# akanazawa/human_dynamics

Measured on AMD Instinct MI355X. Metric: frames/sec/GPU (ResNet+temporal+SMPL, 224x224); SMPL verts max-abs-err, higher is better.
Workload: dtype f16x3

## Files before the change

human_dynamics_amd/_lib.py:

```python
from __future__ import annotations

import ctypes as C
import os

from . import devflags

HERE = os.path.dirname(os.path.abspath(__file__))
LIB_PATH = devflags.get("LIB_PATH") or os.path.join(HERE, "libhmmr_hip.so")

HMMR_F32, HMMR_BF16, HMMR_F16X3 = 0, 1, 2
FLAG_SATURATED = 1
FLAG_NAN = 2
ABI_VERSION = 19
RESNET_UNITS = 16
RESNET_PROF_SLOTS = 64
MAX_TEMPORAL_BLOCKS = 8
MAX_REGRESSORS = 8

_vp, _fp, _ip = C.c_void_p, C.c_void_p, C.c_void_p


class ConvDesc(C.Structure):
    _fields_ = [
        ("in_", _vp), ("w", _vp), ("scale", _fp), ("shift", _fp), ("res", _vp), ("out", _vp),
# ... 2 lines not shown
        ("n_img", C.c_int), ("hin", C.c_int), ("win", C.c_int), ("cin", C.c_int),
        ("in_img_stride", C.c_int64), ("in_row_stride", C.c_int), ("in_px_stride", C.c_int),
        ("kh", C.c_int), ("kw", C.c_int), ("sy", C.c_int), ("sx", C.c_int), ("py", C.c_int), ("px", C.c_int),
        ("ho", C.c_int), ("wo", C.c_int), ("cout", C.c_int), ("ldo", C.c_int),
        ("ldr", C.c_int), ("res_strided", C.c_int), ("res_img_stride", C.c_int64),
        ("res_row_stride", C.c_int), ("res_px_stride", C.c_int),
        ("relu", C.c_int), ("tile", C.c_int),
        ("split_k", C.c_int), ("ws", _vp), ("ws_bytes", C.c_size_t),
        ("pro_scale", _fp), ("pro_shift", _fp),
        ("out_b", _vp), ("ldo_b", C.c_int), ("n_split", C.c_int), ("relu_b", C.c_int),
        ("in2", _vp), ("cin2", C.c_int), ("k_order", C.c_int),
        ("batch", C.c_int), ("batch_in_bytes", C.c_int64), ("batch_w_bytes", C.c_int64), ("batch_out_bytes", C.c_int64),
        ("batch_res_bytes", C.c_int64), ("batch_scale_bytes", C.c_int64), ("batch_shift_bytes", C.c_int64),
    ]


class TailDesc(C.Structure):
    _fields_ = [
        ("dtype", C.c_int), ("h2", _vp), ("m", C.c_int), ("c_mid", C.c_int), ("depth", C.c_int),
        ("w3", _vp), ("scale3", _fp), ("shift3", _fp),
        ("res", _vp), ("ldr", C.c_int), ("res_strided", C.c_int), ("res_img_stride", C.c_int64),
        ("res_row_stride", C.c_int), ("res_px_stride", C.c_int), ("ho", C.c_int), ("wo", C.c_int),
        ("out", _vp), ("pre_scale", _fp), ("pre_shift", _fp),
        ("w1", _vp), ("scale1", _fp), ("shift1", _fp), ("relu1", C.c_int), ("n2", C.c_int),
        ("out_h1", _vp),
        ("h1", _vp), ("hin", C.c_int), ("win", C.c_int), ("w2", _vp), ("scale2", _fp), ("shift2", _fp),
        ("xp", _vp), ("wsc", _vp), ("shift_sc", _fp),
        ("conv2_stride", C.c_int), ("out_pre", _vp),
        ("pair_stream", _vp), ("c_xp", C.c_int), ("unit_stream", _vp),
    ]


class Debug(C.Structure):
    _fields_ = [("stem_route", C.c_int), ("stem_no_conv1", C.c_int), ("gemm_probe", C.c_int), ("smpl_blend_mfma", C.c_int), ("ief_no_group", C.c_int), ("reserved", C.c_int * 3),
                ("pair_min_pixels", C.c_int), ("pair_two_tile_min", C.c_int), ("pair_form", C.c_int)]


class LaunchCounts(C.Structure):
    _fields_ = [("unit_pair", C.c_ulonglong), ("b1_unit", C.c_ulonglong), ("tail_split", C.c_ulonglong), ("conv3x3_stream", C.c_ulonglong),
                ("conv1x1_stream", C.c_ulonglong)]


class Layer(C.Structure):
    _fields_ = [("w", _vp), ("scale", _fp), ("shift", _fp), ("tile", C.c_int), ("k_order", C.c_int)]


class ResnetUnit(C.Structure):
    _fields_ = [("conv1", Layer), ("conv2", Layer), ("conv3", Layer), ("shortcut", Layer), ("c3sc", Layer), ("sc_c1", Layer),
                ("w3_frag", _vp), ("w1n_frag", _vp), ("pair_stream", _vp), ("conv1_frag", _vp), ("unit_stream", _vp), ("pre_scale", _fp), ("pre_shift", _fp),
                ("c_in", C.c_int), ("base", C.c_int), ("depth", C.c_int), ("stride", C.c_int),
                ("fuse_preact", C.c_int), ("fuse_tail", C.c_int)]


class ResnetWeights(C.Structure):
    _fields_ = [("dtype", C.c_int), ("stem", Layer),
                ("unit", ResnetUnit * RESNET_UNITS), ("post_scale", _fp), ("post_shift", _fp)]


class TemporalBlock(C.Structure):
    _fields_ = [("gn1_gamma", _fp), ("gn1_beta", _fp), ("conv1", Layer),
                ("gn2_gamma", _fp), ("gn2_beta", _fp), ("conv2", Layer)]


class TemporalWeights(C.Structure):
    _fields_ = [("dtype", C.c_int), ("num_blocks", C.c_int), ("block", TemporalBlock * MAX_TEMPORAL_BLOCKS)]


# ... 142 lines not shown
```

human_dynamics_amd/csrc/conv3x3_stream.hip:

```cpp
#include <type_traits>

#include "common.h"
#include "hmmr_hip.h"

namespace {

typedef const __attribute__((address_space(1))) void* gptr_t;
typedef __attribute__((address_space(3))) void* lptr_t;

__device__ u32x4 g_s3_dump[64 + 32];

struct S3Args {
    const char* in;
    const char* wstream;
    const float* scale; const float* shift;
    void* out; int ldo;
    int M, H, W, C, nc;
    int relu, tiles_n, n_tiles;
    long long nt_stride;
    unsigned long long* ts;
};

#ifndef S3_PROBE_BITS
#define S3_PROBE_BITS 0
#endif
#define S3_PROBE(bit) (((S3_PROBE_BITS) & (bit)) != 0)
#ifdef HMMR_GEMM_PROBE
#define S3_STAMP(k) do { if (a.ts) { const unsigned long long t_ = __builtin_amdgcn_s_memtime(); if ((threadIdx.x & 63) == 0) a.ts[(blockIdx.x * 4 + (threadIdx.x >> 6)) * 8 + (k)] = t_; } } while (0)
#else
#define S3_STAMP(k) do { } while (0)
#endif

template <int N> __device__ __forceinline__ void s3_wait() {
    static_assert(N >= 0 && N < 64, "vmcnt is a 6-bit counter");
    __builtin_amdgcn_s_waitcnt((N & 15) | (7 << 4) | (0 << 8) | ((N >> 4) << 14));
}

template <int OFF> __device__ __forceinline__ shalf8 s3_rd(unsigned addr) {
    shalf8 v; asm volatile("ds_read_b128 %0, %1 offset:%2" : "=v"(v) : "v"(addr), "n"(OFF)); return v;
}

struct xfrag { shalf8 hi, lo; };

constexpr int S3_NS = 6;

template <int V> using s3_ic = std::integral_constant<int, V>;

template <int FM, int FN, int WGM, int WGN, int WMAX, bool SPLIT = true>
__global__ __launch_bounds__(256, 1) void conv3x3_stream_kernel(const S3Args a) {
    constexpr int NP = SPLIT ? 3 : 2;
    constexpr int ESZ = SPLIT ? 4 : 2;
    constexpr int NB = WGN * FN;
    static_assert(WGM * WGN == 4 && (NB == 4 || NB == 2) && FM * FN <= 16, "4 waves, 128 or 64 channels, at most 16 accumulators");
    constexpr int R = WGM * FM, BM = 32 * R;
    constexpr int NPP = (BM + 2 * WMAX + 2 + 63) / 64;
    constexpr int NS = S3_NS, SLAB = NB * 2048, RING = NS * SLAB;
    constexpr int RW = NB / 2;
    constexpr int ZROWS = 32 * (FM - 1) + 16;
    constexpr int PBUF = (NPP * 64 + ZROWS) * 64;
    constexpr int NR = 2 * (FM + FN), NG = NP * FM * FN;
    static_assert(2048 * (FM - 1) + 16 < 65536, "instruction offsets");
    static_assert(NR <= NG - 4, "one fragment read per gap");

    extern __shared__ __attribute__((aligned(256))) char smem[];
    S3_STAMP(0);
    const int tid = threadIdx.x, lane = tid & 63;
    const int wave = __builtin_amdgcn_readfirstlane(tid >> 6);
    const int lr = lane & 31, lh = lane >> 5;
    const int L = xcd_remap(blockIdx.x, a.n_tiles);
    const int mt = L / a.tiles_n, nt = L - mt * a.tiles_n;
    const int m0 = mt * BM;
    const int W = a.W, HW = a.H * a.W;
    const int base = m0 - W - 1;
    const int nc = a.nc, nk = 9 * nc;
    const int wm = wave / WGN, wn = wave - wm * WGN;
    const unsigned lds0 = (unsigned)(unsigned long long)(lptr_t)smem;

    const char* pptr[NPP];
#pragma unroll
    for (int q = 0; q < NPP; ++q) {
        const int r = 64 * q + 16 * wave + (lane >> 2);
        int px = base + r;
        px = px < 0 ? 0 : (px >= a.M ? a.M - 1 : px);
        pptr[q] = a.in + ((long long)px * a.C) * ESZ + (((lane & 3) ^ ((r >> 2) & 3)) << 4);
        if (S3_PROBE(128)) pptr[q] = a.in + ((long long)(px & ~15) * a.C) * ESZ + lane * 16;
    }
    auto patch_piece = [&](int q, int c, int buf) {
        char* dst = smem + RING + buf * PBUF + wave * 1024;
        __builtin_amdgcn_global_load_lds((gptr_t)(pptr[q] + c * 64), (lptr_t)(dst + q * 4096), 16, 0, 0);
    };
    const char* gw = a.wstream + (long long)nt * a.nt_stride + wave * (RW * 1024) + lane * 16;
    auto ring_dma = [&](int s, int slot) {
        const char* src = gw + (long long)s * SLAB;
        char* dst = smem + slot * SLAB + wave * (RW * 1024);
        __builtin_amdgcn_global_load_lds((gptr_t)src, (lptr_t)dst, 16, 0, 0);
        if constexpr (RW == 2) __builtin_amdgcn_global_load_lds((gptr_t)src, (lptr_t)dst, 16, 1024, 0);
    };
#pragma unroll
    for (int q = 0; q < NPP; ++q) patch_piece(q, 0, 0);
#pragma unroll
    for (int s_ = 0; s_ < NS; ++s_) ring_dma(s_, s_);

    for (int i = tid; i < 2 * ZROWS * 4; i += 256) {
        const int pl = i / (ZROWS * 4), o = i - pl * (ZROWS * 4);
        *(u32x4*)(smem + RING + pl * PBUF + NPP * 64 * 64 + o * 16) = u32x4{0u, 0u, 0u, 0u};
    }
    {
        float* cst = (float*)(smem + RING + 2 * PBUF);
        if (tid < 64 * NB) cst[tid] = tid < 32 * NB ? a.scale[nt * (32 * NB) + tid] : a.shift[nt * (32 * NB) + tid - 32 * NB];
    }
    unsigned mtop[FM], mbot[FM], mlef[FM], mrig[FM];
#pragma unroll
    for (int i = 0; i < FM; ++i) {
        const int m = m0 + (wm * FM + i) * 32 + lr;
        const int rem = m % HW, y = rem / W, x = rem - y * W;
        mtop[i] = (unsigned)__builtin_amdgcn_ballot_w64(y == 0);
        mbot[i] = (unsigned)__builtin_amdgcn_ballot_w64(y == a.H - 1);
        mlef[i] = (unsigned)__builtin_amdgcn_ballot_w64(x == 0);
        mrig[i] = (unsigned)__builtin_amdgcn_ballot_w64(x == W - 1);
    }

    f32x16 acc[FM][FN];
#pragma unroll
    for (int i = 0; i < FM; ++i)
#pragma unroll
        for (int j = 0; j < FN; ++j) {
#pragma unroll
            for (int r = 0; r < 16; ++r) acc[i][j][r] = 0.f;
            asm volatile("" : "+a"(acc[i][j]));
        }

    const unsigned vW = lds0 + wn * FN * 2048 + lane * 16;
    const int rb0 = wm * FM * 32 + lr;
    const unsigned lh2 = SPLIT ? 2 * lh : lh;
    constexpr unsigned XL = SPLIT ? 16u : 32u;
    xfrag fx[2][FM];
    wfrag fw[2][FN];
    unsigned A0 = 0, A0l = 0, Zb = 0, Zbl = 0, adcur = 0, adcurl = 0;

    auto read_one = [&](auto tap_c, int set, int r, int slot_) {
        constexpr int TAP_ = decltype(tap_c)::value, KY = TAP_ / 3, KX = TAP_ % 3;
        if (r < 2 * FN) {
            const int j = r >> 1, pl = r & 1;
#define S3_F(SL, J, PL) if (slot_ == SL && j == J && pl == PL) { shalf8 v = s3_rd<SL * SLAB + J * 2048 + PL * 1024>(vW); if (PL) fw[set][J].lo = v; else fw[set][J].hi = v; }
#define S3_FJ(SL, J) S3_F(SL, J, 0) S3_F(SL, J, 1)
#define S3_FS(SL) S3_FJ(SL, 0) if constexpr (FN > 1) { S3_FJ(SL, 1) } if constexpr (FN > 2) { S3_FJ(SL, 2) S3_FJ(SL, 3) }
            S3_FS(0) S3_FS(1) S3_FS(2) S3_FS(3) S3_FS(4) S3_FS(5)
#undef S3_FS
#undef S3_FJ
#undef S3_F
        } else {
            const int i = (r - 2 * FN) >> 1, pl = (r - 2 * FN) & 1;
            if (pl == 0) {
                if (KY == 1 && KX == 1) { adcur = A0; adcurl = A0l; }
                else {
                    const int ii = i < FM ? i : 0;
                    const unsigned my = KY == 0 ? mtop[ii] : (KY == 2 ? mbot[ii] : 0u);
                    const unsigned mx = KX == 0 ? mlef[ii] : (KX == 2 ? mrig[ii] : 0u);
                    asm volatile("s_mov_b32 vcc_lo, %2\n\ts_mov_b32 vcc_hi, %2\n\tv_cndmask_b32 %0, %3, %4, vcc\n\tv_cndmask_b32 %1, %5, %6, vcc"
                                 : "=&v"(adcur), "=v"(adcurl) : "s"(my | mx), "v"(A0), "v"(Zb), "v"(A0l), "v"(Zbl) : "vcc");
                }
            }
#define S3_X(I) if constexpr (I < FM) { if (i == I) { if (pl) fx[set][I].lo = s3_rd<I * 2048>(adcurl); else fx[set][I].hi = s3_rd<I * 2048>(adcur); } }
            S3_X(0) S3_X(1) S3_X(2) S3_X(3) S3_X(4) S3_X(5) S3_X(6) S3_X(7) S3_X(8) S3_X(9) S3_X(10) S3_X(11) S3_X(12) S3_X(13) S3_X(14) S3_X(15)
#undef S3_X
        }
    };
    auto tap_setup = [&](auto tap_c, int buf_) {
        constexpr int TAP_ = decltype(tap_c)::value, KY = TAP_ / 3, KX = TAP_ % 3;
        const unsigned rowp = (unsigned)(rb0 + KY * W + KX);
        const unsigned ph = (lh2 ^ ((rowp >> 2) & 3u)) << 4;
        const unsigned pb = lds0 + RING + buf_ * PBUF;
        A0 = pb + rowp * 64 + ph;
        A0l = A0 ^ XL;
        Zb = pb + NPP * 64 * 64 + (rowp & 3u) * 64 + ph;
        Zbl = Zb ^ XL;
    };

    __builtin_amdgcn_sched_barrier(0);
    s3_wait<RW * (NS - 1)>();
    __builtin_amdgcn_s_barrier();
    __builtin_amdgcn_sched_barrier(0);
    tap_setup(s3_ic<0>{}, 0);
#pragma unroll
    for (int r = 0; r < NR; ++r) read_one(s3_ic<0>{}, 0, r, 0);
    __builtin_amdgcn_sched_barrier(0);
    s3_wait<RW * (NS - 2)>();
    __builtin_amdgcn_s_barrier();
    __builtin_amdgcn_sched_barrier(0);
    S3_STAMP(1);

    auto step = [&](auto s_c, int kt, int c) {
        constexpr int S = decltype(s_c)::value, TAP = S % 9, SUB = S % NS, CUR = S & 1, NXT = CUR ^ 1;
        constexpr int S1 = (S + 1) % 18, TAP1 = S1 % 9, SNEXT = S1 % NS, BUF1 = S1 / 9, BUFP = (S / 9) ^ 1;
        const bool more = kt + NS < nk;
        const bool pat = TAP == 0 && c + 1 < nc;
#pragma unroll
        for (int i = 0; i < FM; ++i)
#pragma unroll
            for (int p = 0; p < NP; ++p)
#pragma unroll
                for (int j = 0; j < FN; ++j) {
                    if constexpr (SPLIT) {
                        const shalf8& wa = p == 1 ? fw[CUR][j].lo : fw[CUR][j].hi;
                        const shalf8& xb = p == 0 ? fx[CUR][i].lo : fx[CUR][i].hi;
                        if (!S3_PROBE(1)) acc[i][j] = mfma_split(wa, xb, acc[i][j]);
                    } else {
                        const shalf8& wa = p ? fw[CUR][j].lo : fw[CUR][j].hi;
                        const shalf8& xb = p ? fx[CUR][i].lo : fx[CUR][i].hi;
                        if (!S3_PROBE(1)) acc[i][j] = __builtin_amdgcn_mfma_f32_32x32x16_bf16(__builtin_bit_cast(bf16x8, wa), __builtin_bit_cast(bf16x8, xb), acc[i][j], 0, 0, 0);
                    }
                    const int g = (NP * i + p) * FN + j;
                    if (g == 0 && more && !S3_PROBE(4)) ring_dma(kt + NS, SUB);
                    if (g == 1 && !S3_PROBE(16)) tap_setup(s3_ic<TAP1>{}, BUF1);
                    if (TAP == 0 && g >= 2 && g < 2 + NPP && pat && !S3_PROBE(4) && !S3_PROBE(64)) patch_piece(g - 2 < NPP ? g - 2 : 0, c + 1, BUFP);
#pragma unroll
                    for (int r = 0; r < NR; ++r)
                        if (2 + (r * (NG - 4)) / NR == g && !S3_PROBE(2)) read_one(s3_ic<TAP1>{}, NXT, r, SNEXT);
                    __builtin_amdgcn_sched_barrier(0);
                }
        if (S3_PROBE(4) || S3_PROBE(32)) __builtin_amdgcn_s_waitcnt(63 | (7 << 4) | (0 << 8) | (3 << 14));
        else if (more) { if (TAP <= 4 && c + 1 < nc && !S3_PROBE(64)) s3_wait<RW * (NS - 2) + NPP>(); else s3_wait<RW * (NS - 2)>(); }
        else s3_wait<0>();
        __builtin_amdgcn_sched_barrier(0);
        if (!S3_PROBE(8)) __builtin_amdgcn_s_barrier();
        __builtin_amdgcn_sched_barrier(0);
    };
    auto chunk_pair = [&](int kt0, int c0, auto... S) { (step(S, kt0 + decltype(S)::value, c0 + decltype(S)::value / 9), ...); };
    for (int c0 = 0; c0 < nc; c0 += 2)
        chunk_pair(18 * (c0 >> 1), c0, s3_ic<0>{}, s3_ic<1>{}, s3_ic<2>{}, s3_ic<3>{}, s3_ic<4>{}, s3_ic<5>{}, s3_ic<6>{}, s3_ic<7>{}, s3_ic<8>{},
                   s3_ic<9>{}, s3_ic<10>{}, s3_ic<11>{}, s3_ic<12>{}, s3_ic<13>{}, s3_ic<14>{}, s3_ic<15>{}, s3_ic<16>{}, s3_ic<17>{});
    S3_STAMP(2);

    char* stg = smem + wave * 8192;
    const int rsub = lane >> 3, pslot = lane & 7, sw = (lr >> 1) & 7;
    const int nb = nt * (32 * NB) + wn * FN * 32;
    const float lo_clamp = a.relu ? 0.f : -HMMR_SPLIT_MAX;
    f32x4 s4[FN][4], b4[FN][4];
    {
        const float* cst = (const float*)(smem + RING + 2 * PBUF) + wn * FN * 32 + 4 * lh;
#pragma unroll
        for (int j = 0; j < FN; ++j)
#pragma unroll
            for (int g = 0; g < 4; ++g) {
                s4[j][g] = *(const f32x4*)(cst + j * 32 + 8 * g);
                b4[j][g] = *(const f32x4*)(cst + 32 * NB + j * 32 + 8 * g);
            }
    }
    if constexpr (SPLIT) {
        float satmax = 0.f;
        int blk = 0;
    #pragma unroll
        for (int i = 0; i < FM; ++i) {
            const int mb = m0 + (wm * FM + i) * 32;
// ... 44 lines not shown
            bf16_t* orow[2];
#pragma unroll
            for (int q = 0; q < 2; ++q) {
                const int r = 16 * q + (lane >> 2), m = mb + r;
                const int ls = (lane & 3) ^ ((r >> 2) & 3);
                orow[q] = m < a.M ? (bf16_t*)a.out + (long long)m * a.ldo + nb + ls * 8 : (bf16_t*)g_s3_dump + lane * 8;
            }
#pragma unroll
            for (int j = 0; j < FN; ++j, ++blk) {
                char* tile = stg + (blk & 1) * 4096;
#pragma unroll
                for (int g = 0; g < 4; ++g) {
                    typedef __attribute__((ext_vector_type(4))) __bf16 bf16x4;
                    bf16x4 o;
#pragma unroll
                    for (int e = 0; e < 4; ++e) {
                        float v = fmaf(acc[i][j][4 * g + e], s4[j][g][e], b4[j][g][e]);
                        if (a.relu) v = fmaxf(v, 0.f);
                        o[e] = (bf16_t)v;
                    }
                    *(bf16x4*)(tile + lr * 64 + ((g ^ ((lr >> 2) & 3)) << 4) + 8 * lh) = o;
                }
                u32x4 xr[2];
#pragma unroll
                for (int q = 0; q < 2; ++q) xr[q] = *(const u32x4*)(tile + q * 1024 + lane * 16);
#pragma unroll
                for (int q = 0; q < 2; ++q) *(u32x4*)(orow[q] + j * 32) = xr[q];
            }
        }
    }
    S3_STAMP(3);
}

template <int FM, int FN, int WGM, int WGN, int WMAX, bool SPLIT>
int launch_s3_t(const S3Args& base, int cout, hipStream_t stream) {
    S3Args a = base;
    constexpr int NB = WGN * FN, BM = 32 * WGM * FM, NPP = (BM + 2 * WMAX + 2 + 63) / 64;
    constexpr int lds = S3_NS * NB * 2048 + 8 * (NPP * 64 + 32 * (FM - 1) + 16) * 16 + 1024;
    static_assert(lds <= 160 * 1024, "LDS");
    a.tiles_n = cout / (32 * NB);
    a.n_tiles = ((a.M + BM - 1) / BM) * a.tiles_n;
    a.nt_stride = (long long)9 * a.nc * (NB * 2048);
    auto kern = conv3x3_stream_kernel<FM, FN, WGM, WGN, WMAX, SPLIT>;
    static DeviceOnce once;
    if (const unsigned long long bit = once.due()) {
        HMMR_CHECK_HIP(hipFuncSetAttribute((const void*)kern, hipFuncAttributeMaxDynamicSharedMemorySize, lds));
        once.mark(bit);
    }
    hipLaunchKernelGGL(kern, dim3((unsigned)a.n_tiles), dim3(256), lds, stream, a);
    HMMR_CHECK_HIP(hipGetLastError());
    return 0;
}

template <int FM, int FN, int WGM, int WGN, int WMAX>
int launch_s3(const S3Args& a, int cout, bool split, hipStream_t stream) {
    return split ? launch_s3_t<FM, FN, WGM, WGN, WMAX, true>(a, cout, stream) : launch_s3_t<FM, FN, WGM, WGN, WMAX, false>(a, cout, stream);
}

}

extern "C" size_t hmmr_conv3x3_stream_bytes(int cin, int cout) {
    return (size_t)(cout / 32) * (size_t)(9 * (cin / 16)) * 2048;
}

int hmmr_conv3x3_stream(const hmmr_conv_desc_t* d, hipStream_t stream) {
    const bool split = d->in_dtype == HMMR_F16X3 && d->out_dtype == HMMR_F16X3;
    HMMR_REQUIRE(split || (d->in_dtype == HMMR_BF16 && d->out_dtype == HMMR_BF16), "hmmr_conv_gemm: k_order 2 is built for split (f16x3) and bf16 tensors");
    HMMR_REQUIRE(split || d->cin % 64 == 0, "hmmr_conv_gemm: k_order 2 with bf16 tensors needs cin %% 64 == 0 (K steps of 32 channels, taken in pairs)");
    HMMR_REQUIRE(d->cin % 32 == 0 && (d->cout % 128 == 0 || d->cout == 64) && d->win <= 56 && d->scale && d->shift,
                 "hmmr_conv_gemm: k_order 2 needs cin %% 32 == 0, cout %% 128 == 0 (or cout = 64), an image at most 56 pixels wide and scale + shift");
    hmmr_count_launch(HMMR_COUNT_CONV3X3_STREAM);
    S3Args a = {};
    a.in = (const char*)d->in; a.wstream = (const char*)d->w; a.scale = d->scale; a.shift = d->shift;
    a.out = d->out; a.ldo = d->ldo;
    a.M = d->n_img * d->ho * d->wo; a.H = d->hin; a.W = d->win; a.C = d->cin; a.nc = split ? d->cin / 16 : d->cin / 32;
    a.relu = d->relu;
// ... 9 lines not shown
        for (const auto& cd : cand) {
            if ((cd[2] != 0) != narrow || ((cd[0] == 21 || cd[0] == 27 || cd[0] == 28) && !split)) continue;
            const long long tiles = ((rbs + cd[1] - 1) / cd[1]) * nts;
            const double cost = (double)((tiles + 255) / 256) * (cd[1] + 1.5);
            if (!tile || cost < best) { tile = cd[0]; best = cost; }
        }
    }
    HMMR_REQUIRE((tile == 19 || tile == 20) == narrow && (!wide || narrow), "hmmr_conv_gemm: k_order 2: tiles 12 .. 18, 21, 27, 28 take cout %% 128 == 0 and images up to 28 pixels wide, "
                 "tiles 19 / 20 cout = 64 and up to 56 (tile %d, cout %d, win %d)", tile, d->cout, d->win);
    switch (tile) {
    case 12: return launch_s3<7, 2, 2, 2, 28>(a, d->cout, split, stream);
    case 13: return launch_s3<4, 2, 2, 2, 28>(a, d->cout, split, stream);
    case 14: return launch_s3<8, 2, 2, 2, 28>(a, d->cout, split, stream);
    case 15: return launch_s3<6, 2, 2, 2, 28>(a, d->cout, split, stream);
    case 16: return launch_s3<5, 2, 2, 2, 28>(a, d->cout, split, stream);
    case 17: return launch_s3<4, 4, 4, 1, 28>(a, d->cout, split, stream);
    case 18: return launch_s3<3, 4, 4, 1, 28>(a, d->cout, split, stream);
    case 19: return launch_s3<5, 2, 4, 1, 56>(a, d->cout, split, stream);
    case 20: return launch_s3<4, 2, 4, 1, 56>(a, d->cout, split, stream);
    case 21:
        HMMR_REQUIRE(split, "hmmr_conv_gemm: k_order 2, tile 21 (7 x 1 accumulators per wave) is built for split tensors: with two MFMAs per step "
                     "the bf16 form has no room for its 16 fragment reads");
        return launch_s3_t<7, 1, 1, 4, 28, true>(a, d->cout, stream);
    case 27:
    case 28:
        HMMR_REQUIRE(split, "hmmr_conv_gemm: k_order 2, tiles 27 / 28 (2 x 2 and 3 x 2 accumulators per wave) are built for split tensors: with two MFMAs "
                     "per step the bf16 form has no room for their fragment reads");
        return tile == 27 ? launch_s3_t<2, 2, 2, 2, 28, true>(a, d->cout, stream) : launch_s3_t<3, 2, 2, 2, 28, true>(a, d->cout, stream);
    default: break;
    }
    hmmr_set_error("hmmr_conv_gemm: k_order 2 runs tiles 12 .. 21, 27 and 28, not %d", tile);
    return -1;
}
```

human_dynamics_amd/csrc/resnet.hip:

```cpp
#include <stdlib.h>

#include <type_traits>

#include "common.h"
#include "hmmr_hip.h"

int hmmr_stem_fused(const float* images, int n_real, int n, const void* wts, const float* wscale, const float* bias,
                    const float* pscale, const float* pshift, void* out, int dtype, hipStream_t s,
                    const void* w1, const float* s1, const float* b1, void* out_h1);

static constexpr int IMG = 224, PADH = 230, PADW = 232;

__global__ void stem_repack_split_kernel(const float* __restrict__ img, bsplit_t* __restrict__ out, long long npairs,
                                         long long n_real) {
    for (long long i = (long long)blockIdx.x * blockDim.x + threadIdx.x; i < npairs;
         i += (long long)gridDim.x * blockDim.x) {
        const int xp = (int)(i % (PADW / 2));
        const long long t = i / (PADW / 2);
        const int y = (int)(t % PADH);
        const long long n = t / PADH;
        float v[8];
#pragma unroll
        for (int e = 0; e < 8; ++e) v[e] = 0.f;
        const int sy = y - 3;
        if (n < n_real && (unsigned)sy < (unsigned)IMG) {
#pragma unroll
            for (int q = 0; q < 2; ++q) {
                const int sx = 2 * xp + q - 3;
                if ((unsigned)sx < (unsigned)IMG) {
                    const float* p = img + ((n * IMG + sy) * IMG + sx) * 3;
                    v[4 * q] = p[0]; v[4 * q + 1] = p[1]; v[4 * q + 2] = p[2];
                }
            }
        }
        store8(out + i * 8, v);
    }
}

template <typename T>
__global__ void stem_repack_kernel(const float* __restrict__ img, T* __restrict__ out, long long npix,
                                   long long n_real) {
    for (long long i = (long long)blockIdx.x * blockDim.x + threadIdx.x; i < npix;
// ... 217 lines not shown
        } else if (sc_in_tail) {
            HMMR_REQUIRE(U.shortcut.w && !U.shortcut.scale && !fused && U.c_in == 64 && U.stride == 1,
                         "resnet: unit %d cannot compute its shortcut inside the tail", u);
            if (prof_mark(pf)) return -2;
        } else if (U.shortcut.w) {
            d = hmmr_conv_desc_t{};
            d.in = xin; d.pro_scale = ps; d.pro_shift = pb;
            d.w = U.shortcut.w; d.scale = U.shortcut.scale; d.shift = U.shortcut.shift; d.tile = U.shortcut.tile;
            d.out = xn; d.in_dtype = d.out_dtype = w->dtype;
            d.n_img = n; d.hin = H; d.win = H; d.cin = U.c_in;
            d.in_img_stride = (int64_t)H * H * U.c_in; d.in_row_stride = H * U.c_in; d.in_px_stride = U.c_in;
            d.kh = d.kw = 1; d.sy = d.sx = U.stride; d.ho = d.wo = Ho; d.cout = U.depth; d.ldo = U.depth;
            if (sc_c1) {
                d.w = U.sc_c1.w; d.scale = U.sc_c1.scale; d.shift = U.sc_c1.shift; d.k_order = U.sc_c1.k_order;
                d.cout = U.depth + U.base; d.out_b = T1; d.ldo_b = U.base; d.n_split = U.depth; d.relu_b = 1;
            }
            if (hmmr_conv_gemm(&d, s)) return -2;
            if (prof_mark(pf)) return -2;
            if (sc_c1) h1_ready = true;
        }
        if (!h1_ready) {
            d = hmmr_conv_desc_t{};
            d.in = xin; d.pro_scale = ps; d.pro_shift = pb;
            d.w = U.conv1.w; d.scale = U.conv1.scale; d.shift = U.conv1.shift; d.relu = 1; d.tile = U.conv1.tile;
            d.k_order = U.conv1.k_order;
            d.out = T1; d.in_dtype = d.out_dtype = w->dtype;
            d.n_img = n; d.hin = H; d.win = H; d.cin = U.c_in;
            d.in_img_stride = (int64_t)H * H * U.c_in; d.in_row_stride = H * U.c_in; d.in_px_stride = U.c_in;
            d.kh = d.kw = 1; d.sy = d.sx = 1; d.ho = d.wo = H; d.cout = U.base; d.ldo = U.base;
            if (hmmr_conv_gemm(&d, s)) return -2;
        }
        if (prof_mark(pf)) return -2;
        const bool conv2_in_tail = fuse_tail >= 2;
        if (!conv2_in_tail) {
            d = hmmr_conv_desc_t{};
            d.in = T1; d.w = U.conv2.w; d.scale = U.conv2.scale; d.shift = U.conv2.shift; d.relu = 1; d.tile = U.conv2.tile;
            d.k_order = U.conv2.k_order;
            d.out = T2; d.in_dtype = d.out_dtype = w->dtype;
            d.n_img = n; d.hin = H; d.win = H; d.cin = U.base;
            d.in_img_stride = (int64_t)H * H * U.base; d.in_row_stride = H * U.base; d.in_px_stride = U.base;
            d.kh = d.kw = 3; d.sy = d.sx = U.stride; d.py = d.px = 1; d.ho = d.wo = Ho; d.cout = U.base; d.ldo = U.base;
            if (hmmr_conv_gemm(&d, s)) return -2;
        }
        if (prof_mark(pf)) return -2;
        d = hmmr_conv_desc_t{};
        d.in = T2; d.w = U.conv3.w; d.scale = U.conv3.scale; d.shift = U.conv3.shift; d.tile = U.conv3.tile;
        d.in_dtype = d.out_dtype = w->dtype;
        d.n_img = n; d.hin = Ho; d.win = Ho; d.cin = U.base;
        d.in_img_stride = (int64_t)Ho * Ho * U.base; d.in_row_stride = Ho * U.base; d.in_px_stride = U.base;
        d.kh = d.kw = 1; d.sy = d.sx = 1; d.ho = d.wo = Ho; d.cout = U.depth; d.ldo = U.depth;
        d.k_order = U.conv3.k_order;
        if (sc_in_c3) { d.w = U.c3sc.w; d.scale = U.c3sc.scale; d.shift = U.c3sc.shift; d.tile = U.c3sc.tile; d.k_order = U.c3sc.k_order; d.in2 = xin; d.cin2 = U.c_in; }
        else if (U.shortcut.w) { d.res = xn; d.ldr = U.depth; }
        else if (U.stride == 1) { d.res = X[cur]; d.ldr = U.depth; }
        else {
            d.res = X[cur]; d.res_strided = 1;
            d.res_img_stride = (int64_t)H * H * U.depth; d.res_row_stride = U.stride * H * U.depth;
            d.res_px_stride = U.stride * U.depth;
        }
        d.out = write_raw ? xn : nullptr;
        if (write_pre) {
            d.out2 = pn; d.scale2 = w->unit[u + 1].pre_scale; d.shift2 = w->unit[u + 1].pre_shift;
            HMMR_REQUIRE(d.scale2 && d.shift2, "resnet: unit %d lacks its preact BN", u + 1);
        }
        h1_ready = false;
        if (fuse_tail == 4) {
            HMMR_REQUIRE(!last && w->dtype == HMMR_BF16 && U.conv2.scale && U.conv2.shift && !U.shortcut.w &&
// ... 83 lines not shown
```

human_dynamics_amd/devflags.py:

```python
from __future__ import annotations

import os

FLAGS = {
    "LIB_PATH": ("", "load this shared object instead of human_dynamics_amd/libhmmr_hip.so (tools/probe_build.sh)"),
    "STEM": ("", "u[nfused] | f[used]: hmmr_debug_t.stem_route"),
    "STEM_C1": ("1", "0: hmmr_debug_t.stem_no_conv1"),
    "GEMM_PROBE": ("0", "hmmr_debug_t.gemm_probe (only the -DHMMR_GEMM_PROBE development build reads the field; results are garbage there)"),
    "RESNET_CHUNK": ("", "encode the batch in sequential chunks of this many frames (heuristic tiles)"),
    "FUSE_PREACT": ("block1,block2,block3,block4", "blocks whose units pre-activate inside the operand staging of conv1 / shortcut"),
    "FUSE_TAIL": ("1", "0 | 1 | block1 | noconv2 | conv2b1 | nosc | nostride2: which fused bottleneck tails the packer marks"),
    "FUSE_SC": ("1", "0 | 1 | all: shortcut + conv1 as one column-split GEMM (1: blocks 3-4)"),
    "PREACT_FIRST": ("0", "1: a block's first unit fuses its pre-activation too"),
    "FOLD_SC": ("", "0 | 1: conv shortcut folded into conv3's K (default: f16x3 only)"),
    "PATCH_3X3": ("2", "the stride-1 3x3 layers of blocks 2-4 (f16x3): 2 = the one-wave-per-SIMD stream kernel (k_order 2), 1 = the 8-wave patch kernels (k_order 1), 0 = tap-major K order and the im2col gather; the three differ by fp32 accumulation rounding"),
    "B1_STREAM": ("0", "1: the conv2 of block1/unit_1 and unit_2 as a launch of the 3x3 stream kernel (64-channel tiles) instead of inside their fused tails (f16x3; measured equal)"),
    "B1_UNIT": ("1", "0: block1/unit_1 and unit_2 as the round-3 LDS-panel tails with conv2 inside (tap-major conv2) instead of the whole-unit kernel of csrc/b1_unit.hip (f16x3; conv2 chunk-major: the two differ by fp32 accumulation rounding)"),
    "STREAM_1X1": ("1", "0: the conv1 of block 4 and of block2/unit_1 and block3/unit_1's shortcut + conv1 as launches of the 8-wave tiles (csrc/gemm_conv.hip) instead of the two-ring stream kernel of csrc/conv1x1_stream.hip (f16x3; the two differ by fp32 accumulation rounding)"),
    "UNIT_PAIR": ("1", "0 | 1 | block2 | block3: the stride-1 units of blocks 2-3 as register-resident unit pairs (csrc/unit_pair.hip; f16x3)"),
    "AUTOTUNE": ("1", "0: no per-layer tile tuning pass (shipped table / library heuristic only)"),
    "TILE_TABLE": ("1", "0: ignore the shipped tile tables (tile_tables.json), tune or fall back to the heuristic"),
    "TILE_CACHE": ("", "json file the tuned tile tables are read from / written to (profiling runs)"),
    "TUNE_TILES": ("5,6,3,1,2,7,8,11,4", "hmmr_conv_desc_t.tile candidates of the tuner"),
    "RESNET_STREAMS": ("2", "contiguous parts a large batch is encoded as, on concurrent streams"),
    "RESNET_PRIORITY": ("-1", "HIP priority of the ResNet side streams"),
    "TAIL_PRIORITY": ("0", "HIP priority of the tail stream (dist.ShardedPredictor)"),
    "STEP_BUFFERS": ("2", "calls in flight of a pipelined ShardedPredictor (record buffers, and encode streams with STEP_STREAMS): 2, or more to try"),
    "STEP_STREAMS": ("1", "0: keep consecutive steps' ResNet passes on one stream (dist.ShardedPredictor)"),
    "STREAM_POISON": ("", "1: evaluation/streaming.py fills a chunk's record buffer with NaN before its tail writes it (a row nobody wrote, or a download that ran early, shows on the host)"),
    "STREAM_TRACE": ("", "1: evaluation/streaming.py prints the host and device timeline of a call"),
}


def get(name):
    default = FLAGS[name][0]
    return os.environ.get("HMMR_" + name, default)


def is_set(name):
    return ("HMMR_" + name) in os.environ and name in FLAGS
```

human_dynamics_amd/engine.py:

```python
from __future__ import annotations

import ctypes as C
import os
import threading
import time

import numpy as np
import torch

from . import _lib as L
from . import assets, devflags, packing

DTYPES = {"f32": L.HMMR_F32, "fp32": L.HMMR_F32, "float32": L.HMMR_F32,
          "bf16": L.HMMR_BF16, "bfloat16": L.HMMR_BF16,
          "f16x3": L.HMMR_F16X3, "split": L.HMMR_F16X3}
DTYPE_NAMES = {L.HMMR_F32: "f32", L.HMMR_BF16: "bf16", L.HMMR_F16X3: "f16x3"}
DEFAULT_DTYPE = "f16x3"
TILE_TABLES = os.path.join(os.path.dirname(os.path.abspath(__file__)), "tile_tables.json")


def set_debug(stem_route=0, stem_no_conv1=0, gemm_probe=0, smpl_blend_mfma=0, ief_no_group=0, pair_min_pixels=0, pair_two_tile_min=0, pair_form=0):
    d = L.Debug()
    d.stem_route, d.stem_no_conv1, d.gemm_probe = int(stem_route), int(stem_no_conv1), int(gemm_probe)
    d.smpl_blend_mfma, d.ief_no_group, d.pair_min_pixels = int(smpl_blend_mfma), int(ief_no_group), int(pair_min_pixels)
    d.pair_two_tile_min, d.pair_form = int(pair_two_tile_min), int(pair_form)
    L.load().hmmr_set_debug(C.byref(d))


def _debug_from_env():
    e = devflags.get("STEM")
    c1 = devflags.get("STEM_C1")
    probe = int(devflags.get("GEMM_PROBE") or 0)
    if e or c1 == "0" or probe or _debug_from_env.was_set:
        set_debug(stem_route={"u": 1, "f": 2}.get(e[:1], 0), stem_no_conv1=int(c1 == "0"), gemm_probe=probe)
        _debug_from_env.was_set = bool(e or c1 == "0" or probe)


_debug_from_env.was_set = False


def _dt(d):
    if isinstance(d, str):
        if d == "bf16x3":
            import warnings
            warnings.warn("dtype 'bf16x3' is now 'f16x3' (split operands with fp16 halves since round 3)", DeprecationWarning, stacklevel=3)
            d = "f16x3"
        if d not in DTYPES:
            raise ValueError("unknown operand mode %r: use one of %s" % (d, ", ".join(sorted(set(DTYPES)))))
        return DTYPES[d]
    return int(d)


class _Workspace(object):

    def __init__(self, device):
        self.device, self.buf = device, None

    def get(self, nbytes):
        if self.buf is None or self.buf.numel() < nbytes:
            self.buf = torch.empty(int(nbytes), dtype=torch.uint8, device=self.device)
        return self.buf


class HmmrEngine(object):

    def __init__(self, weights, smpl, dtype=DEFAULT_DTYPE, device="cuda:0", num_conv_layers=3,
                 delta_t_values=(-5, 5), joint_type="cocoplus", resnet_chunk=0,
                 temporal_dtype=None, ief_dtype=None, autotune=True, fold_sc=None, fuse_tail=None, patch_3x3=None,
# ... 615 lines not shown
```

include/hmmr_hip.h:

```cpp
#ifndef HMMR_HIP_H
#define HMMR_HIP_H

#include <stddef.h>
#include <stdint.h>

#ifdef __cplusplus
extern "C" {
#endif

#define HMMR_ABI_VERSION 19

enum { HMMR_F32 = 0, HMMR_BF16 = 1, HMMR_F16X3 = 2 };

int hmmr_abi_version(void);
const char* hmmr_last_error(void);

#define HMMR_FLAG_SATURATED 1u
#define HMMR_FLAG_NAN 2u
int hmmr_run_flags(unsigned* flags, int clear);

typedef struct hmmr_debug_s {
    int stem_route;
    int stem_no_conv1;
    int gemm_probe;
    int smpl_blend_mfma;
    int ief_no_group;
    int reserved[3];
    int pair_min_pixels;
    int pair_two_tile_min;
    int pair_form;
} hmmr_debug_t;
void hmmr_set_debug(const hmmr_debug_t* d);
void hmmr_get_debug(hmmr_debug_t* d);

typedef struct {
    unsigned long long unit_pair;
    unsigned long long b1_unit;
    unsigned long long tail_split;
    unsigned long long conv3x3_stream;
    unsigned long long conv1x1_stream;
} hmmr_launch_counts_t;
void hmmr_launch_counts(hmmr_launch_counts_t* out, int clear);

typedef struct {
    const void* in;
    const void* w;
    const float* scale;
    const float* shift;
    const void* res;
    void* out;
    void* out2;
    const float* scale2;
    const float* shift2;
    int in_dtype;
    int out_dtype;
    int n_img, hin, win, cin;
    int64_t in_img_stride;
    int in_row_stride, in_px_stride;
    int kh, kw, sy, sx, py, px;
    int ho, wo;
// ... 266 lines not shown
```

Baseline: 38620.

## Route stride-2 bottleneck conv2 through a stride-2 variant of the streaming conv kernel

Adds a stride-2 mode to the streaming 3x3 conv kernel. It stages two column phases of the input patch for alternating rows, reorders taps so each patch buffer is consumed in turn, and pulls weights straight from the layer weight bank with hand-tuned vmcnt waits. By default, the f16x3 conv2 of the stride-2 ResNet units now goes through this kernel instead of the generic conv GEMM, with a small cost model picking the tile shape. The aim is to bring the pipelined DMA/MFMA schedule to the strided layers. The hand-counted waits and the shifted phase addressing risk subtle correctness issues, and accumulation order changes slightly.

```diff
diff --git a/human_dynamics_amd/_lib.py b/human_dynamics_amd/_lib.py
--- a/human_dynamics_amd/_lib.py
+++ b/human_dynamics_amd/_lib.py
@@ -58,7 +58,7 @@
 
 
 class Debug(C.Structure):
-    _fields_ = [("stem_route", C.c_int), ("stem_no_conv1", C.c_int), ("gemm_probe", C.c_int), ("smpl_blend_mfma", C.c_int), ("ief_no_group", C.c_int), ("reserved", C.c_int * 3),
+    _fields_ = [("stem_route", C.c_int), ("stem_no_conv1", C.c_int), ("gemm_probe", C.c_int), ("smpl_blend_mfma", C.c_int), ("ief_no_group", C.c_int), ("reserved", C.c_int * 2), ("s2_route", C.c_int),
                 ("pair_min_pixels", C.c_int), ("pair_two_tile_min", C.c_int), ("pair_form", C.c_int)]
 
 
diff --git a/human_dynamics_amd/csrc/conv3x3_stream.hip b/human_dynamics_amd/csrc/conv3x3_stream.hip
--- a/human_dynamics_amd/csrc/conv3x3_stream.hip
+++ b/human_dynamics_amd/csrc/conv3x3_stream.hip
@@ -18,6 +18,8 @@
     int M, H, W, C, nc;
     int relu, tiles_n, n_tiles;
     long long nt_stride;
+    const char* wbank; long long ldw;
+    int Hin, Win;
     unsigned long long* ts;
 };
 
@@ -46,21 +48,26 @@
 
 template <int V> using s3_ic = std::integral_constant<int, V>;
 
-template <int FM, int FN, int WGM, int WGN, int WMAX, bool SPLIT = true>
+template <int FM, int FN, int WGM, int WGN, int WMAX, bool SPLIT = true, bool S2 = false>
 __global__ __launch_bounds__(256, 1) void conv3x3_stream_kernel(const S3Args a) {
     constexpr int NP = SPLIT ? 3 : 2;
     constexpr int ESZ = SPLIT ? 4 : 2;
     constexpr int NB = WGN * FN;
     static_assert(WGM * WGN == 4 && (NB == 4 || NB == 2) && FM * FN <= 16, "4 waves, 128 or 64 channels, at most 16 accumulators");
     constexpr int R = WGM * FM, BM = 32 * R;
-    constexpr int NPP = (BM + 2 * WMAX + 2 + 63) / 64;
+    constexpr int NPP = S2 ? (BM + WMAX + 1 + 63) / 64 : (BM + 2 * WMAX + 2 + 63) / 64;
+    constexpr int PHB = NPP * 64 * 64;
+    constexpr int NPH = S2 ? 2 : 1;
+    constexpr int PP = NPH * NPP;
     constexpr int NS = S3_NS, SLAB = NB * 2048, RING = NS * SLAB;
     constexpr int RW = NB / 2;
     constexpr int ZROWS = 32 * (FM - 1) + 16;
-    constexpr int PBUF = (NPP * 64 + ZROWS) * 64;
+    constexpr int PBUF = NPH * PHB + ZROWS * 64;
     constexpr int NR = 2 * (FM + FN), NG = NP * FM * FN;
     static_assert(2048 * (FM - 1) + 16 < 65536, "instruction offsets");
     static_assert(NR <= NG - 4, "one fragment read per gap");
+    static_assert(!S2 || (SPLIT && PP + 2 <= NG && 4 * RW + 2 * PP < 64), "S2: split operands, a buffer's requests one per gap, vmcnt");
+    constexpr int ORD[9] = {0, 1, 2, 6, 7, 8, 3, 4, 5};
 
     extern __shared__ __attribute__((aligned(256))) char smem[];
     S3_STAMP(0);
@@ -82,12 +89,22 @@
         const int r = 64 * q + 16 * wave + (lane >> 2);
         int px = base + r;
         px = px < 0 ? 0 : (px >= a.M ? a.M - 1 : px);
-        pptr[q] = a.in + ((long long)px * a.C) * ESZ + (((lane & 3) ^ ((r >> 2) & 3)) << 4);
+        if constexpr (S2) {
+            const int n_ = px / HW, rem = px - n_ * HW, y_ = rem / W, x_ = rem - y_ * W;
+            px = (n_ * a.Hin + 2 * y_) * a.Win + 2 * x_;
+        }
+        pptr[q] =a.in + ((long long)px * a.C) * ESZ + (((lane & 3) ^ ((r >> 2) & 3)) << 4);
         if (S3_PROBE(128)) pptr[q] = a.in + ((long long)(px & ~15) * a.C) * ESZ + lane * 16;
     }
     auto patch_piece = [&](int q, int c, int buf) {
         char* dst = smem + RING + buf * PBUF + wave * 1024;
         __builtin_amdgcn_global_load_lds((gptr_t)(pptr[q] + c * 64), (lptr_t)(dst + q * 4096), 16, 0, 0);
+    };
+    const long long prow = (long long)a.Win * a.C * ESZ, pcol = (long long)a.C * ESZ;
+    auto patch_piece2 = [&](int i, int c, int buf) {
+        const int ph = i / NPP, q = i - ph * NPP;
+        char* dst = smem + RING + buf * PBUF + ph * PHB + wave * 1024 + q * 4096;
+        __builtin_amdgcn_global_load_lds((gptr_t)(pptr[q] + (1 - buf) * prow + ph * pcol + c * 64), (lptr_t)dst, 16, 0, 0);
     };
     const char* gw = a.wstream + (long long)nt * a.nt_stride + wave * (RW * 1024) + lane * 16;
     auto ring_dma = [&](int s, int slot) {
@@ -96,14 +113,32 @@
         __builtin_amdgcn_global_load_lds((gptr_t)src, (lptr_t)dst, 16, 0, 0);
         if constexpr (RW == 2) __builtin_amdgcn_global_load_lds((gptr_t)src, (lptr_t)dst, 16, 1024, 0);
     };
-#pragma unroll
-    for (int q = 0; q < NPP; ++q) patch_piece(q, 0, 0);
-#pragma unroll
-    for (int s_ = 0; s_ < NS; ++s_) ring_dma(s_, s_);
+    const int jw = RW == 2 ? wave : wave >> 1, plw = RW == 2 ? 0 : wave & 1;
+    const char* gb = S2 ? a.wbank + (long long)(nt * (32 * NB) + 32 * jw + lr) * a.ldw + lh * 32 + plw * 16 : nullptr;
+    auto ring_dma2 = [&](auto t_c, int c, int slot) {
+        const char* src = gb + (long long)(ORD[decltype(t_c)::value] * a.C + 16 * c) * 4;
+        char* dst = smem + slot * SLAB + wave * (RW * 1024);
+        __builtin_amdgcn_global_load_lds((gptr_t)src, (lptr_t)dst, 16, 0, 0);
+        if constexpr (RW == 2) __builtin_amdgcn_global_load_lds((gptr_t)(src + 16), (lptr_t)(dst + 1024), 16, 0, 0);
+    };
+    if constexpr (S2) {
+        static_assert(S3_NS == 6, "the S2 prologue issues six K steps");
+#pragma unroll
+        for (int i = 0; i < PP; ++i) patch_piece2(i, 0, 0);
+#pragma unroll
+        for (int i = 0; i < PP; ++i) patch_piece2(i, 0, 1);
+        ring_dma2(s3_ic<0>{}, 0, 0); ring_dma2(s3_ic<1>{}, 0, 1); ring_dma2(s3_ic<2>{}, 0, 2);
+        ring_dma2(s3_ic<3>{}, 0, 3); ring_dma2(s3_ic<4>{}, 0, 4); ring_dma2(s3_ic<5>{}, 0, 5);
+    } else {
+#pragma unroll
+        for (int q = 0; q < NPP; ++q) patch_piece(q, 0, 0);
+#pragma unroll
+        for (int s_ = 0; s_ < NS; ++s_) ring_dma(s_, s_);
+    }
 
     for (int i = tid; i < 2 * ZROWS * 4; i += 256) {
         const int pl = i / (ZROWS * 4), o = i - pl * (ZROWS * 4);
-        *(u32x4*)(smem + RING + pl * PBUF + NPP * 64 * 64 + o * 16) = u32x4{0u, 0u, 0u, 0u};
+        *(u32x4*)(smem + RING + pl * PBUF + NPH * PHB + o * 16) = u32x4{0u, 0u, 0u, 0u};
     }
     {
         float* cst = (float*)(smem + RING + 2 * PBUF);
@@ -152,11 +187,11 @@
         } else {
             const int i = (r - 2 * FN) >> 1, pl = (r - 2 * FN) & 1;
             if (pl == 0) {
-                if (KY == 1 && KX == 1) { adcur = A0; adcurl = A0l; }
+                if (S2 ? (KY != 0 && KX != 0) : (KY == 1 && KX == 1)) { adcur = A0; adcurl = A0l; }
                 else {
                     const int ii = i < FM ? i : 0;
-                    const unsigned my = KY == 0 ? mtop[ii] : (KY == 2 ? mbot[ii] : 0u);
-                    const unsigned mx = KX == 0 ? mlef[ii] : (KX == 2 ? mrig[ii] : 0u);
+                    const unsigned my = KY == 0 ? mtop[ii] : (KY == 2 && !S2 ? mbot[ii] : 0u);
+                    const unsigned mx = KX == 0 ? mlef[ii] : (KX == 2 && !S2 ? mrig[ii] : 0u);
                     asm volatile("s_mov_b32 vcc_lo, %2\n\ts_mov_b32 vcc_hi, %2\n\tv_cndmask_b32 %0, %3, %4, vcc\n\tv_cndmask_b32 %1, %5, %6, vcc"
                                  : "=&v"(adcur), "=v"(adcurl) : "s"(my | mx), "v"(A0), "v"(Zb), "v"(A0l), "v"(Zbl) : "vcc");
                 }
@@ -168,12 +203,13 @@
     };
     auto tap_setup = [&](auto tap_c, int buf_) {
         constexpr int TAP_ = decltype(tap_c)::value, KY = TAP_ / 3, KX = TAP_ % 3;
-        const unsigned rowp = (unsigned)(rb0 + KY * W + KX);
+        constexpr int RY = S2 ? (KY == 0 ? 0 : 1) : KY, RX = S2 ? (KX == 0 ? 0 : 1) : KX, PHO = S2 && KX != 1 ? PHB : 0;
+        const unsigned rowp = (unsigned)(rb0 + RY * W + RX);
         const unsigned ph = (lh2 ^ ((rowp >> 2) & 3u)) << 4;
         const unsigned pb = lds0 + RING + buf_ * PBUF;
-        A0 = pb + rowp * 64 + ph;
+        A0 = pb + PHO + rowp * 64 + ph;
         A0l = A0 ^ XL;
-        Zb = pb + NPP * 64 * 64 + (rowp & 3u) * 64 + ph;
+        Zb = pb + NPH * PHB + (rowp & 3u) * 64 + ph;
         Zbl = Zb ^ XL;
     };
 
@@ -191,10 +227,13 @@
     S3_STAMP(1);
 
     auto step = [&](auto s_c, int kt, int c) {
-        constexpr int S = decltype(s_c)::value, TAP = S % 9, SUB = S % NS, CUR = S & 1, NXT = CUR ^ 1;
-        constexpr int S1 = (S + 1) % 18, TAP1 = S1 % 9, SNEXT = S1 % NS, BUF1 = S1 / 9, BUFP = (S / 9) ^ 1;
+        constexpr int S = decltype(s_c)::value, T = S % 9, SUB = S % NS, CUR = S & 1, NXT = CUR ^ 1;
+        constexpr int S1 = (S + 1) % 18, T1 = S1 % 9, SNEXT = S1 % NS, BUFP = (S / 9) ^ 1;
+        constexpr int TAP = S2 ? ORD[T] : T, TAP1 = S2 ? ORD[T1] : T1, BUF1 = S2 ? (T1 < 6 ? 0 : 1) : S1 / 9;
+        constexpr int GRING = S2 && T == 5 ? NG - 1 : 0;
         const bool more = kt + NS < nk;
         const bool pat = TAP == 0 && c + 1 < nc;
+        const bool nxt = c + 1 < nc;
 #pragma unroll
         for (int i = 0; i < FM; ++i)
 #pragma unroll
@@ -211,15 +250,27 @@
                         if (!S3_PROBE(1)) acc[i][j] = __builtin_amdgcn_mfma_f32_32x32x16_bf16(__builtin_bit_cast(bf16x8, wa), __builtin_bit_cast(bf16x8, xb), acc[i][j], 0, 0, 0);
                     }
                     const int g = (NP * i + p) * FN + j;
-                    if (g == 0 && more && !S3_PROBE(4)) ring_dma(kt + NS, SUB);
+                    if constexpr (S2) {
+                        if ((T == 5 || T == 8) && g >= 2 && g < 2 + PP && nxt) patch_piece2(g - 2 < PP ? g - 2 : 0, c + 1, T == 5 ? 0 : 1);
+                        if (g == GRING && more) ring_dma2(s3_ic<(S + NS) % 9>{}, c + ((S + NS) / 9 - S / 9), SUB);
+                    } else {
+                        if (g == 0 && more && !S3_PROBE(4)) ring_dma(kt + NS, SUB);
+                    }
                     if (g == 1 && !S3_PROBE(16)) tap_setup(s3_ic<TAP1>{}, BUF1);
-                    if (TAP == 0 && g >= 2 && g < 2 + NPP && pat && !S3_PROBE(4) && !S3_PROBE(64)) patch_piece(g - 2 < NPP ? g - 2 : 0, c + 1, BUFP);
+                    if (!S2 && TAP == 0 && g >= 2 && g < 2 + NPP && pat && !S3_PROBE(4) && !S3_PROBE(64)) patch_piece(g - 2 < NPP ? g - 2 : 0, c + 1, BUFP);
 #pragma unroll
                     for (int r = 0; r < NR; ++r)
                         if (2 + (r * (NG - 4)) / NR == g && !S3_PROBE(2)) read_one(s3_ic<TAP1>{}, NXT, r, SNEXT);
                     __builtin_amdgcn_sched_barrier(0);
                 }
-        if (S3_PROBE(4) || S3_PROBE(32)) __builtin_amdgcn_s_waitcnt(63 | (7 << 4) | (0 << 8) | (3 << 14));
+        if constexpr (S2) {
+            if (!more) s3_wait<0>();
+            else if constexpr (T <= 3) { if (c > 0) s3_wait<4 * RW + PP>(); else s3_wait<4 * RW>(); }
+            else if constexpr (T == 4) s3_wait<4 * RW>();
+            else if constexpr (T <= 6) { if (nxt) s3_wait<4 * RW + PP>(); else s3_wait<4 * RW>(); }
+            else if constexpr (T == 7) { if (nxt) s3_wait<3 * RW>(); else s3_wait<4 * RW>(); }
+            else { if (nxt) s3_wait<4 * RW + 2 * PP>(); else s3_wait<4 * RW>(); }
+        } else if (S3_PROBE(4) || S3_PROBE(32)) __builtin_amdgcn_s_waitcnt(63 | (7 << 4) | (0 << 8) | (3 << 14));
         else if (more) { if (TAP <= 4 && c + 1 < nc && !S3_PROBE(64)) s3_wait<RW * (NS - 2) + NPP>(); else s3_wait<RW * (NS - 2)>(); }
         else s3_wait<0>();
         __builtin_amdgcn_sched_barrier(0);
@@ -330,16 +381,16 @@
     S3_STAMP(3);
 }
 
-template <int FM, int FN, int WGM, int WGN, int WMAX, bool SPLIT>
+template <int FM, int FN, int WGM, int WGN, int WMAX, bool SPLIT, bool S2 = false>
 int launch_s3_t(const S3Args& base, int cout, hipStream_t stream) {
     S3Args a = base;
-    constexpr int NB = WGN * FN, BM = 32 * WGM * FM, NPP = (BM + 2 * WMAX + 2 + 63) / 64;
-    constexpr int lds = S3_NS * NB * 2048 + 8 * (NPP * 64 + 32 * (FM - 1) + 16) * 16 + 1024;
+    constexpr int NB = WGN * FN, BM = 32 * WGM * FM, NPP = S2 ? (BM + WMAX + 1 + 63) / 64 : (BM + 2 * WMAX + 2 + 63) / 64;
+    constexpr int lds = S3_NS * NB * 2048 + 2 * ((S2 ? 2 : 1) * NPP * 64 + 32 * (FM - 1) + 16) * 64 + 1024;
     static_assert(lds <= 160 * 1024, "LDS");
     a.tiles_n = cout / (32 * NB);
     a.n_tiles = ((a.M + BM - 1) / BM) * a.tiles_n;
     a.nt_stride = (long long)9 * a.nc * (NB * 2048);
-    auto kern = conv3x3_stream_kernel<FM, FN, WGM, WGN, WMAX, SPLIT>;
+    auto kern = conv3x3_stream_kernel<FM, FN, WGM, WGN, WMAX, SPLIT, S2>;
     static DeviceOnce once;
     if (const unsigned long long bit = once.due()) {
         HMMR_CHECK_HIP(hipFuncSetAttribute((const void*)kern, hipFuncAttributeMaxDynamicSharedMemorySize, lds));
@@ -415,3 +466,33 @@
     hmmr_set_error("hmmr_conv_gemm: k_order 2 runs tiles 12 .. 21, 27 and 28, not %d", tile);
     return -1;
 }
+
+int hmmr_conv3x3_s2_stream(const void* in, const hmmr_layer_t* L, void* out, int n_img, int hin, int cin, int cout, hipStream_t stream) {
+    HMMR_REQUIRE(in && L && L->w && L->scale && L->shift && out && n_img > 0, "hmmr_conv3x3_s2_stream: null argument");
+    const bool narrow = cout == 64;
+    const int ho = hin / 2;
+    HMMR_REQUIRE(hin % 2 == 0 && cin % 32 == 0 && (narrow || cout % 128 == 0) && ho <= (narrow ? 28 : 14),
+                 "hmmr_conv3x3_s2_stream: needs an even image, cin %% 32 == 0 and cout = 64 (images up to 56 wide) or cout %% 128 == 0 (up to 28) "
+                 "(hin %d, cin %d, cout %d)", hin, cin, cout);
+    S3Args a = {};
+    a.in = (const char*)in; a.wbank = (const char*)L->w; a.ldw = (long long)9 * cin * 4;
+    a.scale = L->scale; a.shift = L->shift; a.out = out; a.ldo = cout;
+    a.M = n_img * ho * ho; a.H = ho; a.W = ho; a.Hin = hin; a.Win = hin; a.C = cin; a.nc = cin / 16;
+    a.relu = 1;
+    static const int cand[4][3] = {{0, 7, 0}, {1, 4, 0}, {3, 8, 1}, {4, 12, 1}};
+    const long long rbs = (a.M + 31) / 32, nts = narrow ? 1 : cout / 128;
+    int pick = -1;
+    double best = 0;
+    for (const auto& cd : cand) {
+        if ((cd[2] != 0) != narrow) continue;
+        const long long tiles = ((rbs + cd[1] - 1) / cd[1]) * nts;
+        const double cost = (double)((tiles + 255) / 256) * (cd[1] + 1.5);
+        if (pick < 0 || cost < best) { pick = cd[0]; best = cost; }
+    }
+    switch (pick) {
+    case 0: return launch_s3_t<7, 1, 1, 4, 14, true, true>(a, cout, stream);
+    case 1: return launch_s3_t<2, 2, 2, 2, 14, true, true>(a, cout, stream);
+    case 3: return launch_s3_t<2, 2, 4, 1, 28, true, true>(a, cout, stream);
+    default: return launch_s3_t<3, 2, 4, 1, 28, true, true>(a, cout, stream);
+    }
+}
diff --git a/human_dynamics_amd/csrc/resnet.hip b/human_dynamics_amd/csrc/resnet.hip
--- a/human_dynamics_amd/csrc/resnet.hip
+++ b/human_dynamics_amd/csrc/resnet.hip
@@ -8,6 +8,8 @@
 int hmmr_stem_fused(const float* images, int n_real, int n, const void* wts, const float* wscale, const float* bias,
                     const float* pscale, const float* pshift, void* out, int dtype, hipStream_t s,
                     const void* w1, const float* s1, const float* b1, void* out_h1);
+
+int hmmr_conv3x3_s2_stream(const void* in, const hmmr_layer_t* L, void* out, int n_img, int hin, int cin, int cout, hipStream_t stream);
 
 static constexpr int IMG = 224, PADH = 230, PADW = 232;
 
@@ -291,7 +293,10 @@
         }
         if (prof_mark(pf)) return -2;
         const bool conv2_in_tail = fuse_tail >= 2;
-        if (!conv2_in_tail) {
+        const bool s2_stream = w->dtype == HMMR_F16X3 && U.stride == 2 && !conv2_in_tail && U.conv2.k_order == 0 && dbg->s2_route == 0;
+        if (s2_stream) {
+            if (hmmr_conv3x3_s2_stream(T1, &U.conv2, T2, n, H, U.base, U.base, s)) return -2;
+        } else if (!conv2_in_tail) {
             d = hmmr_conv_desc_t{};
             d.in = T1; d.w = U.conv2.w; d.scale = U.conv2.scale; d.shift = U.conv2.shift; d.relu = 1; d.tile = U.conv2.tile;
             d.k_order = U.conv2.k_order;
diff --git a/human_dynamics_amd/devflags.py b/human_dynamics_amd/devflags.py
--- a/human_dynamics_amd/devflags.py
+++ b/human_dynamics_amd/devflags.py
@@ -7,6 +7,7 @@
     "STEM": ("", "u[nfused] | f[used]: hmmr_debug_t.stem_route"),
     "STEM_C1": ("1", "0: hmmr_debug_t.stem_no_conv1"),
     "GEMM_PROBE": ("0", "hmmr_debug_t.gemm_probe (only the -DHMMR_GEMM_PROBE development build reads the field; results are garbage there)"),
+    "S2_ROUTE": ("0", "1: hmmr_debug_t.s2_route = 1, the f16x3 conv2 of the stride-2 units through hmmr_conv_gemm instead of the stride-2 stream kernel (differ by fp32 accumulation rounding)"),
     "RESNET_CHUNK": ("", "encode the batch in sequential chunks of this many frames (heuristic tiles)"),
     "FUSE_PREACT": ("block1,block2,block3,block4", "blocks whose units pre-activate inside the operand staging of conv1 / shortcut"),
     "FUSE_TAIL": ("1", "0 | 1 | block1 | noconv2 | conv2b1 | nosc | nostride2: which fused bottleneck tails the packer marks"),
diff --git a/human_dynamics_amd/engine.py b/human_dynamics_amd/engine.py
--- a/human_dynamics_amd/engine.py
+++ b/human_dynamics_amd/engine.py
@@ -19,11 +19,12 @@
 TILE_TABLES = os.path.join(os.path.dirname(os.path.abspath(__file__)), "tile_tables.json")
 
 
-def set_debug(stem_route=0, stem_no_conv1=0, gemm_probe=0, smpl_blend_mfma=0, ief_no_group=0, pair_min_pixels=0, pair_two_tile_min=0, pair_form=0):
+def set_debug(stem_route=0, stem_no_conv1=0, gemm_probe=0, smpl_blend_mfma=0, ief_no_group=0, pair_min_pixels=0, pair_two_tile_min=0, pair_form=0,
+              s2_route=0):
     d = L.Debug()
     d.stem_route, d.stem_no_conv1, d.gemm_probe = int(stem_route), int(stem_no_conv1), int(gemm_probe)
     d.smpl_blend_mfma, d.ief_no_group, d.pair_min_pixels = int(smpl_blend_mfma), int(ief_no_group), int(pair_min_pixels)
-    d.pair_two_tile_min, d.pair_form = int(pair_two_tile_min), int(pair_form)
+    d.pair_two_tile_min, d.pair_form, d.s2_route = int(pair_two_tile_min), int(pair_form), int(s2_route)
     L.load().hmmr_set_debug(C.byref(d))
 
 
@@ -31,9 +32,10 @@
     e = devflags.get("STEM")
     c1 = devflags.get("STEM_C1")
     probe = int(devflags.get("GEMM_PROBE") or 0)
-    if e or c1 == "0" or probe or _debug_from_env.was_set:
-        set_debug(stem_route={"u": 1, "f": 2}.get(e[:1], 0), stem_no_conv1=int(c1 == "0"), gemm_probe=probe)
-        _debug_from_env.was_set = bool(e or c1 == "0" or probe)
+    s2 = int(devflags.get("S2_ROUTE") or 0)
+    if e or c1 == "0" or probe or s2 or _debug_from_env.was_set:
+        set_debug(stem_route={"u": 1, "f": 2}.get(e[:1], 0), stem_no_conv1=int(c1 == "0"), gemm_probe=probe, s2_route=s2)
+        _debug_from_env.was_set = bool(e or c1 == "0" or probe or s2)
 
 
 _debug_from_env.was_set = False
diff --git a/include/hmmr_hip.h b/include/hmmr_hip.h
--- a/include/hmmr_hip.h
+++ b/include/hmmr_hip.h
@@ -25,7 +25,8 @@
     int gemm_probe;
     int smpl_blend_mfma;
     int ief_no_group;
-    int reserved[3];
+    int reserved[2];
+    int s2_route;
     int pair_min_pixels;
     int pair_two_tile_min;
     int pair_form;
```

Measured after the change: 38850 (median of 6 runs). Within noise of the previous version (+0.6%).
